# jedbrown/spectral-petsc

Measured on NVIDIA B200. Metric: spectral MatMult GDOF/s (fp64), higher is better.
Workload: dtype f64

## Files before the change

### spectral_petsc_b200/csrc/elliptic.cu

```cuda
#include "elliptic.h"

#include <algorithm>
#include <cmath>
#include <cstdlib>
#include <vector>

#include "../../include/spectral_b200.h"
#include "cheb_matrix.h"
#include "common.cuh"
#include "deriv.h"

namespace sb200 {

namespace {

struct LineInfo {
  bool interior;
  long long gid0;
  long long did0;
};

__device__ __forceinline__ LineInfo decode_line(const GridDesc& gd, long long line) {
  const int d = gd.d, PL = gd.dim[d - 1];
  long long rem = line, cnt = -gd.goff;
// ... 169 lines not shown
int GridDesc::init_slab(int d_, const int* dim_global, int rank, int nranks) {
  SB_TRY(init(d_, dim_global));
  if (nranks == 1) return 0;
  SB_CHECK(d >= 2, SB200_ERR_USER, "slab partition needs at least two axes");
  SB_CHECK(dim[0] % nranks == 0, SB200_ERR_USER, "slab partition: the outermost extent must be divisible by the number of ranks");
  const int nloc = dim[0] / nranks;
  n0g = dim[0];
  i0 = rank * nloc;
  dim[0] = nloc;
  m = (long long)nloc * stride[0];
  const int lo = i0 < 1 ? 1 : i0, hi = (i0 + nloc > n0g - 1) ? n0g - 1 : i0 + nloc;
  g = (long long)(hi > lo ? hi - lo : 0) * istride[0];
  goff = (long long)(lo - 1) * istride[0];
  return 0;
}

int EllipticCtx::create(int d, const int* dim, int rank, int nranks, EllipticCtx** out) {
  EllipticCtx* e = new EllipticCtx();
  int rc = e->init(d, dim, rank, nranks);
  if (rc) {
    delete e;
    return rc;
  }
  *out = e;
  return 0;
}

int EllipticCtx::init(int d, const int* dim, int rank, int nranks) {
  SB_TRY(gd.init_slab(d, dim, rank, nranks));
  gtot = 1;
  for (int k = 0; k < d; k++) {
    gdim[k] = dim[k];
    gtot *= dim[k] - 2;
  }
  nw = 2 + d;
  const size_t mb = (size_t)gd.m * sizeof(double);
  const int narr = nw + d + 2 + (nranks > 1 ? 6 : 0);
  SB_TRY(arena.init((size_t)narr * (mb + 256), rank, nranks));
  for (int k = 0; k < nw; k++) SB_CHECK((w[k] = arena.alloc_doubles(gd.m)), SB200_ERR_CUDA, "arena exhausted");
  for (int k = 0; k < d; k++) {
    SB_CHECK((gradu[k] = arena.alloc_doubles(gd.m)), SB200_ERR_CUDA, "arena exhausted");
    SB_CUDA(cudaMemset(gradu[k], 0, mb));
  }
  SB_CHECK((eta = arena.alloc_doubles(gd.m)), SB200_ERR_CUDA, "arena exhausted");
  SB_CHECK((deta = arena.alloc_doubles(gd.m)), SB200_ERR_CUDA, "arena exhausted");
  if (nranks > 1) {
    SB_CHECK((eta_p = arena.alloc_doubles(gd.m)), SB200_ERR_CUDA, "arena exhausted");
    SB_CHECK((deta_p = arena.alloc_doubles(gd.m)), SB200_ERR_CUDA, "arena exhausted");
    SB_CHECK((g0_p = arena.alloc_doubles(gd.m)), SB200_ERR_CUDA, "arena exhausted");
    SB_CHECK((Wp = arena.alloc_doubles(gd.m)), SB200_ERR_CUDA, "arena exhausted");
    SB_CHECK((Xp = arena.alloc_doubles(gd.m)), SB200_ERR_CUDA, "arena exhausted");
    SB_CHECK((Yp = arena.alloc_doubles(gd.m)), SB200_ERR_CUDA, "arena exhausted");
  }
  SB_CUDA(cudaMalloc((void**)&sync, 512));
  SB_CUDA(cudaMemset(sync, 0, 512));
  SB_CUDA(cudaMalloc((void**)&dirichlet, std::max<size_t>(8, (size_t)(gd.m - gd.g) * sizeof(double))));
  SB_CUDA(cudaMemset(dirichlet, 0, std::max<size_t>(8, (size_t)(gd.m - gd.g) * sizeof(double))));
  SB_CUDA(cudaMalloc((void**)&b, std::max<size_t>(8, (size_t)gd.g * sizeof(double))));
  SB_CUDA(cudaMemset(b, 0, std::max<size_t>(8, (size_t)gd.g * sizeof(double))));
  {
    std::vector<double> ones((size_t)gd.m, 1.0);
    SB_CUDA(cudaMemcpy(eta, ones.data(), mb, cudaMemcpyHostToDevice));
    SB_CUDA(cudaMemset(deta, 0, mb));
  }
  for (int k = 0; k < d; k++) {
    Dax[k] = nullptr;
    for (int q = 0; q < k; q++)
      if (gdim[q] == gdim[k]) Dax[k] = Dax[q];
    if (!Dax[k]) {
      DiffMatrix* dm = new DiffMatrix();
      SB_TRY(DiffMatrix::create(gdim[k], dm));
      owned.push_back(dm);
      Dax[k] = dm;
    }
  }
  return 0;
}

EllipticCtx::~EllipticCtx() {
  free_slab_maps(tmaps);
  arena.destroy();
  if (dirichlet) cudaFree(dirichlet);
  if (b) cudaFree(b);
  if (sync) cudaFree(sync);
  if (gexec) {
    cudaDeviceSynchronize();
    cudaGraphExecDestroy(gexec);
  }
  if (gstream) cudaStreamDestroy(gstream);
  if (gU) cudaFree(gU);
  if (gV) cudaFree(gV);
  for (DiffMatrix* dm : owned) {
    dm->destroy();
    delete dm;
  }
}

bool EllipticCtx::fusable() const {
  static int use = -1;
  if (use < 0) {
    const char* c = getenv("SB200_NO_EO");
    const char* f = getenv("SB200_NO_FUSE");
    use = ((c && atoi(c)) || (f && atoi(f))) ? 0 : 1;
  }
  if (!use || arena.nranks > 1 || gd.d > SB200_EO_MAX_JOBS) return false;
  for (int k = 0; k < gd.d; k++)
    if (!deriv_eo_supported(job(k, w[0], w[1], nullptr, DERIV_STORE))) return false;
  return true;
// ... 66 lines not shown
  p.O = gd.m / (gd.stride[axis] * gd.dim[axis]);
  p.R = gd.stride[axis];
  p.xs = p.ys = 1;
  p.xoff = p.yoff = 0;
  p.mode = mode;
  if (axis == 0 && arena.nranks > 1) {
    SB_CHECK(arena.attached(), SB200_ERR_USER, "slab partition: peers are not attached (exchange the IPC handles first)");
    if (slab_deriv0_pencil_supported(arena, p)) return slab_deriv0_pencil(arena, p, gd.dim[0], gd.i0, Xp, Yp, s);
    p.npeer = arena.nranks;
    p.nloc = gd.dim[0];
    p.row0 = gd.i0;
    for (int q = 0; q < arena.nranks; q++) p.xpeer[q] = arena.on(q, x);
    SB_TRY(arena.barrier(s));
    SB_TRY(deriv_apply(p, s));
    return arena.barrier(s);
  }
  return deriv_apply(p, s);
}

int EllipticCtx::pad(const double* U, bool with_dirichlet, double* local, cudaStream_t s) {
  const int PL = gd.dim[gd.d - 1];
  const long long nlines = gd.m / PL;
  const int tx = 32;
  dim3 blk(tx, 256 / tx);
  pad_kernel<<<(unsigned)((nlines + blk.y - 1) / blk.y), blk, 0, s>>>(gd, nlines, U, with_dirichlet ? dirichlet : nullptr, local);
  count_launch();
  SB_CUDA(cudaGetLastError());
  return 0;
}

int EllipticCtx::crop(const double* local, const double* rhs, double* V, cudaStream_t s) {
  const int PL = gd.dim[gd.d - 1];
  const long long nlines = gd.m / PL;
  const int tx = PL >= 128 ? 128 : (PL > 32 ? 64 : 32);
  dim3 blk(tx, 256 / tx);
  crop_kernel<<<(unsigned)((nlines + blk.y - 1) / blk.y), blk, 0, s>>>(gd, nlines, local, rhs, V);
  count_launch();
  SB_CUDA(cudaGetLastError());
  return 0;
}

int EllipticCtx::matmult(const double* U, double* V, cudaStream_t s) {
  SB_CHECK(U && V && U != V, SB200_ERR_ARG, "MatMult_Elliptic: U and V must be distinct non-null vectors");
  if (arena.nranks > 1) {
    SB_CHECK(arena.attached(), SB200_ERR_USER, "slab partition: peers are not attached (exchange the IPC handles first)");
    SB_CHECK(!arena.failed(), SB200_ERR_CUDA, "slab partition: a device-side flag wait timed out earlier (a peer never arrived or the ranks' calls went out of step); results are undefined, the context refuses further work");
    if ((path == 0 || path == 3) && elliptic_slab_fused_supported(*this)) {
      last_kernel = "slab step: stage_kernel + persist_kernel<P,8,1,SLAB> per rank (axis-0 chain on pencils exchanged through NVLink peer memory)";
      return elliptic_matmult_slab_fused(*this, U, V, s);
    }
    SB_CHECK(path <= 1, SB200_ERR_SUP, "slab partition: the fused path needs equal extents P in {32,64,128}");
  } else if (path == 3 || (path == 0 && elliptic_persist_supported(*this))) {
    SB_CHECK(elliptic_persist_supported(*this), SB200_ERR_SUP, "persistent path needs equal extents P % 16 == 0 between 32 and 160");
    last_kernel = "persist_kernel<P,NWARPS,1> phases A+B (the whole MatMult step: 2 PDL-linked launches)";
    return elliptic_matmult_persist(*this, U, V, s);
  }
  if (path == 2 && arena.nranks == 1) {
    SB_CHECK(elliptic_fused_supported(*this), SB200_ERR_SUP, "fused path needs equal extents P in {32,64,128}");
    last_kernel = "chain_kernel per axis";
    return elliptic_matmult_fused(*this, U, V, s);
  }
  if (path == 4 && arena.nranks == 1) {
    last_kernel = "generic path replayed from a CUDA graph";
    return matmult_graph(U, V, s);
  }
  last_kernel = "generic path: pad + per-axis deriv_kernel / eo_deriv_kernel + pointwise kernels";
  return matmult_generic(U, V, s);
}

int EllipticCtx::matmult_graph(const double* U, double* V, cudaStream_t s) {
  const size_t bytes = (size_t)gd.g * sizeof(double);
  if (!gexec) {
    if (!gU) SB_CUDA(cudaMalloc((void**)&gU, bytes));
    if (!gV) SB_CUDA(cudaMalloc((void**)&gV, bytes));
    if (!gstream) SB_CUDA(cudaStreamCreateWithFlags(&gstream, cudaStreamNonBlocking));
    SB_CUDA(cudaStreamSynchronize(s));
    SB_CUDA(cudaMemsetAsync(gU, 0, bytes, gstream));
    SB_TRY(matmult_generic(gU, gV, gstream));
    SB_CUDA(cudaStreamSynchronize(gstream));
    SB_CUDA(cudaStreamBeginCapture(gstream, cudaStreamCaptureModeThreadLocal));
    const int rc = matmult_generic(gU, gV, gstream);
    cudaGraph_t graph = nullptr;
    const cudaError_t ce = cudaStreamEndCapture(gstream, &graph);
    if (rc || ce != cudaSuccess || !graph) {
      if (graph) cudaGraphDestroy(graph);
      cudaGetLastError();
      SB_CHECK(rc == 0, rc, "MatMult_Elliptic: the generic path failed while being captured");
      set_last_error(std::string("cudaStreamEndCapture: ") + cudaGetErrorString(ce));
      return SB200_ERR_CUDA;
    }
    size_t nn = 0;
    cudaGraphGetNodes(graph, nullptr, &nn);
    gnodes = (int)nn;
    const cudaError_t ie = cudaGraphInstantiate(&gexec, graph, 0);
    cudaGraphDestroy(graph);
    SB_CUDA(ie);
  }
  SB_CUDA(cudaMemcpyAsync(gU, U, bytes, cudaMemcpyDeviceToDevice, s));
  SB_CUDA(cudaGraphLaunch(gexec, s));
  SB_CUDA(cudaMemcpyAsync(V, gV, bytes, cudaMemcpyDeviceToDevice, s));
  count_launch(gnodes);
  return 0;
}

int EllipticCtx::matmult_generic(const double* U, double* V, cudaStream_t s) {
  const int d = gd.d;
  if (fusable()) {
// ... 69 lines not shown
```

### spectral_petsc_b200/csrc/elliptic.h

```cpp
#pragma once
#include <cuda_runtime.h>

#include <vector>

#include "symm.h"

#define SB200_MAX_DIM 10
#define SB200_EO_MAX_P 160

namespace sb200 {

struct DiffMatrix {
  int P = 0, Pp = 0;
  double* d_D = nullptr;
  double* d_Ae = nullptr;
  double* d_Bo = nullptr;
  int HP = 0;
  double* d_Aep = nullptr;
  double* d_Bop = nullptr;
  static int create(int P, DiffMatrix* out);
  void destroy();
};

struct GridDesc {
  int d;
  int dim[SB200_MAX_DIM];
  long long stride[SB200_MAX_DIM];
  long long istride[SB200_MAX_DIM];
  long long m, g;
  int i0, n0g;
  long long goff;
  int init(int d, const int* dim);
  int init_slab(int d, const int* dim_global, int rank, int nranks);
  __host__ __device__ int gext(int j) const { return j == 0 ? n0g : dim[j]; }
  __host__ __device__ int gidx(int j, int i) const { return j == 0 ? i + i0 : i; }
};

struct EllipticCtx {
  GridDesc gd;
  int nw = 0;
  double* w[SB200_MAX_DIM + 2] = {};
  double* gradu[SB200_MAX_DIM] = {};
  double* eta = nullptr;
  double* deta = nullptr;
  double* dirichlet = nullptr;
  double* b = nullptr;
  double gamma = 0.0, exponent = 2.0;
  int path = 0;
  const char* last_kernel = "none";
  long long* trace = nullptr;
  unsigned* sync = nullptr;
  DiffMatrix* Dax[SB200_MAX_DIM] = {};
  std::vector<DiffMatrix*> owned;
  SymmArena arena;
  int gdim[SB200_MAX_DIM] = {};
  long long gtot = 0;
  double* Wp = nullptr;
  double* eta_p = nullptr;
  double* deta_p = nullptr;
  double* g0_p = nullptr;
  double* Xp = nullptr;
  double* Yp = nullptr;
  bool pencil_valid = false;
  unsigned long long mm_epoch = 0;
  struct SlabMaps* tmaps = nullptr;
  bool tmaps_tried = false;

  static int create(int d, const int* dim, int rank, int nranks, EllipticCtx** out);
  int init(int d, const int* dim, int rank, int nranks);
  ~EllipticCtx();
  int refresh_pencils(cudaStream_t s);
  int deriv(int axis, const double* x, double* y, const double* yin, int mode, cudaStream_t s);
  bool fusable() const;
  struct EoLineMap line_map(int axis) const;
  struct DerivParams job(int axis, const double* x, double* y, const double* yin, int mode) const;
// ... 25 lines not shown
```

### spectral_petsc_b200/csrc/elliptic_persist.cu

```cuda
#include <cstdlib>

#include "../../include/spectral_b200.h"
#include "chain.cuh"
#include "deriv.h"
#include "elliptic.h"
#include "persist.h"

#ifdef SB200_ABLATE
#define XF(p, bit) (((p).xflags & (bit)) != 0)
#else
#define XF(p, bit) false
#endif

#ifdef SB200_TRACE
#define STAMP(k) do { if (lane == 0 && p.trace) tr[k] = clock64(); } while (0)
#else
#define STAMP(k) do { } while (0)
#endif

namespace sb200 {

namespace {

__device__ __forceinline__ unsigned long long gtime() {
  unsigned long long t;
  asm volatile("mov.u64 %0, %%globaltimer;" : "=l"(t));
  return t;
}
__device__ __forceinline__ void tl_stamp(const PersistParams& p, int slot) {
  if (!XF(p, 64) || p.epoch != p.tl_epoch) return;
  unsigned long long* ts = reinterpret_cast<unsigned long long*>(p.sync) + 16;
  const unsigned long long t = gtime();
  atomicMin(ts + 2 * slot, t);
  atomicMax(ts + 2 * slot + 1, t);
}


template <int P, int NT, bool RIGHT>
__device__ __forceinline__ void load_item(double* Xw, const double* __restrict__ U, int d, int axis,
                                          long long n0, int lane, const SlabGeom sg) {
  constexpr int BE = RIGHT ? EO<P>::BLOCK_ELEMS_RIGHT : EO<P>::BLOCK_ELEMS_LEFT;
#pragma unroll
  for (int j = 0; j < NT; j++) load_block_from_U<P, RIGHT>(Xw + j * BE, U, d, axis, (unsigned)(n0 + 8 * j), lane, sg);
}

struct FluxBuf {
  double2 e[2][2], de[2][2], gg[2][2];
};

template <int P, bool RIGHT>
__device__ __forceinline__ void flux_load(FluxBuf& f, const Own<P, RIGHT>& own, int ib, const double* __restrict__ eta,
                                          const double* __restrict__ deta, const double* __restrict__ g0) {
#pragma unroll
  for (int ii = 0; ii < 2; ii++) {
    if (ib + ii >= EO<P>::MT) continue;
    if (eta == nullptr) {
      f.e[ii][0] = f.e[ii][1] = make_double2(1.5, 1.5);
      f.de[ii][0] = f.de[ii][1] = f.gg[ii][0] = f.gg[ii][1] = make_double2(0.25, 0.25);
      continue;
    }
    const long long ot = own.top(ib + ii), ob = own.bot(ib + ii);
    f.e[ii][0] = ldg2(eta + ot);
    f.e[ii][1] = ldg2(eta + ob);
    f.de[ii][0] = ldg2(deta + ot);
    f.de[ii][1] = ldg2(deta + ob);
    f.gg[ii][0] = ldg2(g0 + ot);
    f.gg[ii][1] = ldg2(g0 + ob);
  }
}

template <int P, bool RIGHT>
__device__ __forceinline__ void flux_apply(const FluxBuf& f, const Own<P, RIGHT>& own, int ib, double* Xj,
                                           const double (&a)[EO<P>::MT][2], const double (&b)[EO<P>::MT][2]) {
#pragma unroll
  for (int ii = 0; ii < 2; ii++) {
    const int i = ib + ii;
    if (i >= EO<P>::MT) continue;
    const int st = own.stop(i), sb = own.sbot(i);
    const double2 wt = ld2(Xj + st), wb = ld2(Xj + sb);
    const double yt0 = a[i][0] + b[i][0], yt1 = a[i][1] + b[i][1];
    const double yb0 = RIGHT ? b[i][1] - a[i][1] : b[i][0] - a[i][0];
    const double yb1 = RIGHT ? b[i][0] - a[i][0] : b[i][1] - a[i][1];
    const double ft0 = __dadd_rn(__dmul_rn(f.e[ii][0].x, yt0), __dmul_rn(__dmul_rn(f.de[ii][0].x, wt.x), f.gg[ii][0].x));
    const double ft1 = __dadd_rn(__dmul_rn(f.e[ii][0].y, yt1), __dmul_rn(__dmul_rn(f.de[ii][0].y, wt.y), f.gg[ii][0].y));
    const double fb0 = __dadd_rn(__dmul_rn(f.e[ii][1].x, yb0), __dmul_rn(__dmul_rn(f.de[ii][1].x, wb.x), f.gg[ii][1].x));
    const double fb1 = __dadd_rn(__dmul_rn(f.e[ii][1].y, yb1), __dmul_rn(__dmul_rn(f.de[ii][1].y, wb.y), f.gg[ii][1].y));
    st2(Xj + st, ft0, ft1);
    st2(Xj + sb, fb0, fb1);
  }
}

__device__ __forceinline__ void tma_store_2d(const CUtensorMap* map, int c0, int c1, const void* smem_src) {
  const unsigned s = (unsigned)__cvta_generic_to_shared(smem_src);
  asm volatile("cp.async.bulk.tensor.2d.global.shared::cta.bulk_group [%0, {%1, %2}], [%3];" ::"l"(map), "r"(c0), "r"(c1), "r"(s) : "memory");
}

struct NoEarly {
  __device__ __forceinline__ void operator()() const {}
};

template <int P, int NT, bool RIGHT, bool DEEP, bool PENCIL = false, bool WAITDONE = false, typename F = NoEarly>
__device__ __forceinline__ void run_item(const PersistParams& p, int axis, long long n0, const double* Ae,
                                         const double* Bo, double* Xw, int lane, const SlabMaps* maps = nullptr, double* stage = nullptr,
                                         F after_gemm2 = F()) {
  using E = EO<P>;
  static_assert(!(PENCIL && RIGHT), "pencil items are strided-axis items");
  constexpr int BE = RIGHT ? E::BLOCK_ELEMS_RIGHT : E::BLOCK_ELEMS_LEFT;
  const int g = lane >> 2, t = lane & 3;
  LineGeom lg;
  lg.R = PENCIL ? p.Rp : p.R[axis];
  lg.PR = (long long)P * lg.R;
  lg.nlines = PENCIL ? p.Rp : p.nlines;
  Own<P, RIGHT> own[NT];
  long long base0[NT];
#pragma unroll
  for (int j = 0; j < NT; j++) {
    const long long nj = n0 + 8 * j;
    base0[j] = RIGHT ? nj * P : lg.base(nj);
    own[j].base = RIGHT ? (nj + g) * P : base0[j] + 2 * t;
    own[j].R = lg.R;
    own[j].g = g;
    own[j].t = t;
  }
  const double* __restrict__ g0 = PENCIL ? p.g0_p : p.g0[axis];
  const double* __restrict__ eta_a = PENCIL ? p.eta_p : p.eta;
  const double* __restrict__ deta_a = PENCIL ? p.deta_p : p.deta;
  const double* __restrict__ etap = XF(p, 1) ? nullptr : eta_a;
#ifdef SB200_TRACE
  long long* tr = p.trace ? p.trace + ((long long)axis * (p.nlines / (8 * NT)) + n0 / (8 * NT)) * 8 : nullptr;
  if (lane == 0 && p.trace) { unsigned smid; asm("mov.u32 %0, %%smid;" : "=r"(smid)); tr[6] = smid; tr[7] = threadIdx.x >> 5; }
#endif
  STAMP(0);
  FluxBuf f0, f1;
  if (DEEP) flux_load<P, RIGHT>(f0, own[0], 0, etap, deta_a, g0);
#pragma unroll
  for (int j = 0; j < NT; j++) {
    prefetch_block<P, RIGHT>(eta_a, base0[j], lg.R, lane);
    prefetch_block<P, RIGHT>(deta_a, base0[j], lg.R, lane);
    prefetch_block<P, RIGHT>(g0, base0[j], lg.R, lane);
    if (RIGHT && !PENCIL) {
      for (int k = 0; k < p.d - 1; k++) prefetch_block<P, true>(p.part[k], base0[j], 1, lane);
    }
  }
  cp_async_wait<0>();
  __syncwarp();
  STAMP(1);

  double a[NT][E::MT][2], b[NT][E::MT][2];
  eo_gemm_nt<P, NT, RIGHT>(Ae, Bo, Xw, a, b, g, t);
// ... 20 lines not shown
    }
  }
  __syncwarp();
  STAMP(3);
  eo_gemm_nt<P, NT, RIGHT>(Ae, Bo, Xw, a, b, g, t);
  __syncwarp();
  after_gemm2();
  STAMP(4);

  if (XF(p, 2)) {
    if (a[0][0][0] + b[0][0][0] == 12345.678) p.V[0] = 1.0;
  } else if (PENCIL && NT == 1 && p.bulk) {
    asm volatile("cp.async.bulk.wait_group.read 0;" ::: "memory");
    __syncwarp();
#pragma unroll
    for (int i = 0; i < E::MT; i++) {
      const int mt = i * 8 + g, mb = P - 1 - mt;
      st2(stage + mt * 8 + 2 * t, a[0][i][0] + b[0][i][0], a[0][i][1] + b[0][i][1]);
      st2(stage + mb * 8 + 2 * t, b[0][i][0] - a[0][i][0], b[0][i][1] - a[0][i][1]);
    }
    asm volatile("fence.proxy.async.shared::cta;" ::: "memory");
    __syncwarp();
    if (lane < p.nranks) {
      const int nloc = 1 << p.lognloc;
      const int col = (int)((long long)p.rank * p.Rp + n0);
      tma_store_2d(&maps->m[lane], col, 0, stage + (lane << p.lognloc) * 8);
    }
    asm volatile("cp.async.bulk.commit_group;" ::: "memory");
  } else if (PENCIL) {
    const int nloc = 1 << p.lognloc;
#pragma unroll
    for (int j = 0; j < NT; j++) {
      const long long col = (long long)p.rank * p.Rp + n0 + 8 * j + 2 * t;
#pragma unroll
      for (int i = 0; i < E::MT; i++) {
        const int mt = i * 8 + g, mb = P - 1 - mt;
        const int qt = XF(p, 16) ? p.rank : mt >> p.lognloc, qb = XF(p, 16) ? p.rank : mb >> p.lognloc;
        st2(p.part0peer[qt] + (long long)(mt - qt * nloc) * p.R0 + col, a[j][i][0] + b[j][i][0], a[j][i][1] + b[j][i][1]);
        st2(p.part0peer[qb] + (long long)(mb - qb * nloc) * p.R0 + col, b[j][i][0] - a[j][i][0], b[j][i][1] - a[j][i][1]);
      }
    }
  } else if (!RIGHT) {
    double* __restrict__ part = p.part[axis];
#pragma unroll
    for (int j = 0; j < NT; j++) {
#pragma unroll
      for (int i = 0; i < E::MT; i++) {
        st2(part + own[j].top(i), a[j][i][0] + b[j][i][0], a[j][i][1] + b[j][i][1]);
        st2(part + own[j].bot(i), b[j][i][0] - a[j][i][0], b[j][i][1] - a[j][i][1]);
      }
    }
  } else {
    asm volatile("griddepcontrol.wait;" ::: "memory");
    if (WAITDONE && p.merged) {
      if (lane == 0) {
        const long long t0 = clock64();
        while (*reinterpret_cast<volatile unsigned*>(p.sync + 6) < p.nlocal_items) {
          if (clock64() - t0 > SB200_SPIN_LIMIT) {
            symm_record_timeout(p.sf.f[p.rank]);
            break;
          }
        }
        __threadfence();
      }
      __syncwarp();
    }
    if (WAITDONE && !XF(p, 8)) {
      if (lane == 0) tl_stamp(p, 6);
      if (lane < p.nranks) spin_until(p.sf.f[p.rank] + SYMM_DONE + lane, p.epoch, p.sf.f[p.rank]);
      __syncwarp();
      if (lane == 0) tl_stamp(p, 7);
    }
#pragma unroll
    for (int j = 0; j < NT; j++) {
      long long n = n0 + 8 * j + g, gid = 0, mul = 1;
      bool vint = true;
      for (int q = p.d - 2; q >= 0; q--) {
        int iq;
        if (q == 0) {
          iq = (int)n + p.sg.i0;
        } else {
          iq = (int)(n % P);
          n /= P;
        }
        const int ext = q == 0 ? p.sg.n0g : P;
        vint = vint && iq > 0 && iq < ext - 1;
        gid += (long long)(iq - 1) * mul;
        mul *= P - 2;
      }
      const long long vrow = gid * (P - 2) - p.sg.goff - 1;
#pragma unroll
      for (int ib = 0; ib < E::MT; ib += 4) {
        double2 ot[4], ob[4];
#pragma unroll
        for (int ii = 0; ii < 4; ii++) ot[ii] = ob[ii] = make_double2(0.0, 0.0);
        if (p.d == 3) {
          double2 lt[2][4], lb[2][4];
#pragma unroll
          for (int k = 0; k < 2; k++) {
            const double* __restrict__ pk = p.part[k];
#pragma unroll
            for (int ii = 0; ii < 4; ii++) {
              if (ib + ii >= E::MT) continue;
              lt[k][ii] = __ldcg(reinterpret_cast<const double2*>(pk + own[j].top(ib + ii)));
              lb[k][ii] = __ldcg(reinterpret_cast<const double2*>(pk + own[j].bot(ib + ii)));
            }
// ... 69 lines not shown
      const bool live = line < l1;
      const unsigned ml = line / lpp, lin = line - ml * lpp;
      unsigned rem = lin;
      long long gid = 0, ist = P - 2;
      bool inter = live;
      for (int j = d - 2; j >= 1; j--) {
        const int ij = (int)(rem % P);
        rem /= P;
        inter = inter && ij >= 1 && ij <= P - 2;
        gid += (long long)(ij - 1) * ist;
        ist *= (P - 2);
      }
      const int i0g = (int)ml + p.sg.i0;
      inter = inter && i0g >= 1 && i0g <= p.sg.n0g - 2;
      gid += (long long)(i0g - 1) * ist - p.sg.goff;
#pragma unroll
      for (int it = 0; it < IT; it++) {
        const int k = 2 * lane + 64 * it;
        v[b][it][0] = (inter && k >= 1 && k <= P - 2) ? U[gid + k - 1] : 0.0;
        v[b][it][1] = (inter && k + 1 <= P - 2) ? U[gid + k] : 0.0;
        const unsigned n = lin * P + k, q = n / Rp;
        dst[b][it] = (live && k < P) ? p.wppeer[q] + (long long)i0g * Rp + (n - q * Rp) : nullptr;
      }
    }
#pragma unroll
    for (int b = 0; b < LB; b++)
#pragma unroll
      for (int it = 0; it < IT; it++)
        if (dst[b][it]) st2(dst[b][it], v[b][it][0], v[b][it][1]);
  }
}

template <int P>
__global__ void __launch_bounds__(128, 6) stage_kernel(PersistParams p) {
  asm volatile("griddepcontrol.launch_dependents;" ::: "memory");
  stage_push_share<P>(p, threadIdx.x >> 5, blockDim.x >> 5);
  if (threadIdx.x == 0) tl_stamp(p, 1);
  __syncthreads();
  if (threadIdx.x == 0) {
    __threadfence_system();
    tl_stamp(p, 2);
    if (atomicAdd(p.sync + 3, 1u) == gridDim.x - 1) {
      p.sync[3] = 0;
      __threadfence_system();
      for (int q = 0; q < p.nranks; q++) st_relaxed_sys(p.sf.f[q] + SYMM_READY + p.rank, p.epoch);
    }
  }
}

constexpr int persist_maxreg(int nwarps, bool slab_a) {
  return nwarps > 8 ? (65536 / (nwarps * 32)) / 8 * 8 : (slab_a ? 216 : 255);
}

template <int P, int NWARPS, int NT, bool LASTPHASE, bool SLAB>
__global__ void __maxnreg__(persist_maxreg(NWARPS, SLAB && !LASTPHASE)) persist_kernel(PersistParams p, const __grid_constant__ SlabMaps maps) {
  using E = EO<P>;
  extern __shared__ __align__(128) double sm[];
  double* Ae = sm;
  double* Bo = sm + E::H * E::LDM;
  constexpr int BEMAX = E::BLOCK_ELEMS_RIGHT > E::BLOCK_ELEMS_LEFT ? E::BLOCK_ELEMS_RIGHT : E::BLOCK_ELEMS_LEFT;
  const int warp = threadIdx.x >> 5, lane = threadIdx.x & 31;
  double* Xw = sm + E::MAT_ELEMS + warp * (NT * BEMAX);
  double* stage = (SLAB && !LASTPHASE) ? sm + E::MAT_ELEMS + NWARPS * (NT * BEMAX) + warp * (P * 8) : nullptr;
  unsigned* sync = p.sync + (LASTPHASE ? 4 : 0);

  const unsigned items_per_axis = (unsigned)(p.nlines / (8 * NT));
  const unsigned items0 = (SLAB && !LASTPHASE) ? (unsigned)(p.Rp / (8 * NT)) : 0u;
  const unsigned nlocal = LASTPHASE ? items_per_axis : items_per_axis * (p.d - 1 - p.first_axis);
  const bool merged = SLAB && !LASTPHASE && p.merged;
  const unsigned total = nlocal + items0 + (merged ? items_per_axis : 0u);
  if (!LASTPHASE) asm volatile("griddepcontrol.launch_dependents;" ::: "memory");

  load_matrices<P>(sm, p.Ae, p.Bo);
  if (SLAB && threadIdx.x == 0) tl_stamp(p, LASTPHASE ? 5 : 0);

  const unsigned nstatic = gridDim.x * NWARPS;
  auto grab = [&]() -> unsigned {
    unsigned tk = 0;
    if (lane == 0) tk = atomicAdd(sync, 1u) + nstatic;
    return __shfl_sync(0xffffffffu, tk, 0);
  };
  const unsigned first_ticket = warp * gridDim.x + blockIdx.x;
  bool peers_ready = false;
  auto issue_load = [&](unsigned tk) {
    if (tk >= total) return;
    if (SLAB && !LASTPHASE && tk >= nlocal + items0) {
      load_item<P, NT, true>(Xw, p.U, p.d, p.d - 1, (long long)(tk - nlocal - items0) * (8 * NT), lane, p.sg);
      return;
    }
    if (SLAB && !LASTPHASE && tk >= nlocal) {
      if (!peers_ready && !XF(p, 4)) {
        if (lane < p.nranks) spin_until(p.sf.f[p.rank] + SYMM_READY + lane, p.epoch, p.sf.f[p.rank]);
        __syncwarp();
        if (lane == 0) tl_stamp(p, 3);
        peers_ready = true;
      }
      LineGeom lg;
      lg.R = p.Rp;
      lg.PR = (long long)P * p.Rp;
      lg.nlines = p.Rp;
#pragma unroll
      for (int j = 0; j < NT; j++)
        load_block<P, false>(Xw + j * E::BLOCK_ELEMS_LEFT, p.Wp, lg, (long long)(tk - nlocal) * (8 * NT) + 8 * j, lane);
      return;
    }
    const unsigned tl = tk;
    const int arel = LASTPHASE ? 0 : tl / items_per_axis;
    const int axis = LASTPHASE ? p.d - 1 : p.first_axis + arel;
    const long long n0 = (long long)(tl - arel * items_per_axis) * (8 * NT);
    load_item<P, NT, LASTPHASE>(Xw, p.U, p.d, axis, n0, lane, p.sg);
  };

  constexpr bool DEEP = (NWARPS * NT <= 8);
  unsigned tk = 0;
  if (SLAB && !LASTPHASE) {
    cp_async_wait<0>();
    __syncthreads();
    tk = first_ticket;
    issue_load(tk);
  } else {
    tk = first_ticket;
    issue_load(tk);
    cp_async_wait<0>();
    __syncthreads();
  }
  if (p.stagger > 0) {
    const long long until = clock64() + (long long)(warp / 4) * p.stagger;
    while (clock64() < until) {
    }
  }

  unsigned pencil_done = 0;
  auto report_pencils = [&]() {
    if (p.bulk) {
      asm volatile("cp.async.bulk.wait_group 0;" ::: "memory");
      asm volatile("fence.proxy.async.global;" ::: "memory");
      __syncwarp();
    }
    __threadfence_system();
    if (lane == 0) {
      const unsigned before = atomicAdd(sync + 2, pencil_done);
      if (before + pencil_done == items0) {
        tl_stamp(p, 4);
        sync[2] = 0;
        __threadfence_system();
        for (int q = 0; q < p.nranks; q++) st_relaxed_sys(p.sf.f[q] + SYMM_DONE + p.rank, p.epoch);
      }
    }
    pencil_done = 0;
  };
  unsigned nxt = 0;
  while (tk < total) {
    if (SLAB && !LASTPHASE && tk >= nlocal + items0) {
      if (pencil_done) report_pencils();
      run_item<P, NT, true, DEEP, false, true>(p, p.d - 1, (long long)(tk - nlocal - items0) * (8 * NT), Ae, Bo, Xw, lane);
    } else if (SLAB && !LASTPHASE && tk >= nlocal) {
      run_item<P, NT, false, DEEP, true>(p, 0, (long long)(tk - nlocal) * (8 * NT), Ae, Bo, Xw, lane, &maps, stage);
      pencil_done++;
    } else {
      const unsigned tl = tk;
      const int arel = LASTPHASE ? 0 : tl / items_per_axis;
      const int axis = LASTPHASE ? p.d - 1 : p.first_axis + arel;
      const long long n0 = (long long)(tl - arel * items_per_axis) * (8 * NT);
      if (SLAB) {
        run_item<P, NT, LASTPHASE, DEEP, false, SLAB && LASTPHASE>(p, axis, n0, Ae, Bo, Xw, lane);
      } else {
        auto early = [&]() {
          nxt = grab();
          issue_load(nxt);
        };
        run_item<P, NT, LASTPHASE, DEEP, false, false>(p, axis, n0, Ae, Bo, Xw, lane, nullptr, nullptr, early);
      }
      if (merged) {
        __threadfence();
        __syncwarp();
        if (lane == 0) atomicAdd(sync + 6, 1u);
      }
    }
    if (SLAB) {
      tk = grab();
      issue_load(tk);
    } else {
      tk = nxt;
    }
  }
  cp_async_wait<0>();
  if (SLAB && !LASTPHASE && pencil_done) report_pencils();
  if (lane == 0) {
    const unsigned gone = atomicAdd(sync + 1, 1u);
    if (gone == gridDim.x * NWARPS - 1) {
      sync[0] = 0;
      sync[1] = 0;
      if (merged) sync[6] = 0;
      if (SLAB) tl_stamp(p, LASTPHASE ? 9 : 8);
    }
  }
}

template <int P, int NWARPS, int NT, bool LASTPHASE, bool SLAB>
int launch_phase(const PersistParams& p, size_t smem, int sms, cudaStream_t s) {
  auto kern = persist_kernel<P, NWARPS, NT, LASTPHASE, SLAB>;
  static bool attr[64] = {};
  int cur = 0;
  cudaGetDevice(&cur);
  if (!attr[cur & 63]) {
    SB_CUDA(cudaFuncSetAttribute(kern, cudaFuncAttributeMaxDynamicSharedMemorySize, (int)smem));
    attr[cur & 63] = true;
  }
  long long items = p.nlines / (8 * NT) * (LASTPHASE ? 1 : p.d - 1 - p.first_axis);
  if (SLAB && !LASTPHASE) items += p.Rp / (8 * NT) + (p.merged ? p.nlines / (8 * NT) : 0);
  if (items <= 0) return 0;
  long long grid = items < sms ? items : sms;
  if (const char* mc = getenv("SB200_MAX_CTAS")) {
    const int lim = atoi(mc);
    if (lim > 0 && grid > lim) grid = lim;
  }
  if (grid < 1) grid = 1;
  cudaLaunchConfig_t cfg = {};
  cfg.gridDim = dim3((unsigned)grid);
  cfg.blockDim = dim3(NWARPS * 32);
  cfg.dynamicSmemBytes = smem;
  cfg.stream = s;
  cudaLaunchAttribute at[1];
  at[0].id = cudaLaunchAttributeProgrammaticStreamSerialization;
  at[0].val.programmaticStreamSerializationAllowed = 1;
  cfg.attrs = at;
  cfg.numAttrs = (LASTPHASE || SLAB) ? 1 : 0;
  static const SlabMaps no_maps = {};
  SB_CUDA(cudaLaunchKernelEx(&cfg, kern, p, (SLAB && p.maps) ? *p.maps : no_maps));
  count_launch();
  return 0;
}

template <int P, int NWARPS, int NT>
int run_cfg(PersistParams& p, cudaStream_t s) {
  using E = EO<P>;
  constexpr int BEMAX = E::BLOCK_ELEMS_RIGHT > E::BLOCK_ELEMS_LEFT ? E::BLOCK_ELEMS_RIGHT : E::BLOCK_ELEMS_LEFT;
  const size_t smem = (size_t)(E::MAT_ELEMS + NWARPS * NT * BEMAX) * sizeof(double);
  const size_t smem_slab_a = smem + (size_t)NWARPS * P * 8 * sizeof(double);
  int dev = 0, sms = 148;
  cudaGetDevice(&dev);
  cudaDeviceGetAttribute(&sms, cudaDevAttrMultiProcessorCount, dev);
  if (p.nranks > 1) {
    if (!XF(p, 32)) {
      int blocks = sms;
      if (const char* mc = getenv("SB200_MAX_CTAS")) blocks = atoi(mc) > 0 ? atoi(mc) : blocks;
      {
        static bool carve[64] = {};
        if (!carve[dev & 63]) {
          cudaFuncSetAttribute(stage_kernel<P>, cudaFuncAttributePreferredSharedMemoryCarveout, cudaSharedmemCarveoutMaxShared);
          carve[dev & 63] = true;
        }
      }
      stage_kernel<P><<<blocks, 128, 0, s>>>(p);
      count_launch();
      SB_CUDA(cudaGetLastError());
    }
    p.nlocal_items = (unsigned)(p.nlines / (8 * NT) * (p.d - 1 - p.first_axis));
    if (NT != 1) p.bulk = 0;
    SB_TRY((launch_phase<P, NWARPS, NT, false, true>(p, smem_slab_a, sms, s)));
    if (!p.merged) SB_TRY((launch_phase<P, NWARPS, NT, true, true>(p, smem, sms, s)));
    return 0;
  }
  SB_TRY((launch_phase<P, NWARPS, NT, false, false>(p, smem, sms, s)));
  SB_TRY((launch_phase<P, NWARPS, NT, true, false>(p, smem, sms, s)));
  return 0;
}

}

bool elliptic_persist_supported(const EllipticCtx& e) {
  const int d = e.gd.d;
  if (d < 2 || e.arena.nranks > 1) return false;
  const int P = e.gd.dim[0];
  for (int j = 1; j < d; j++)
    if (e.gd.dim[j] != P) return false;
  return P % 16 == 0 && P >= 32 && P <= 160 && (e.gd.m / P) % 16 == 0;
}

int persist_run(int P, PersistParams& p, cudaStream_t s) {
  static int cfg = -1, stg = -1;
  if (cfg < 0) {
    const char* c = getenv("SB200_PERSIST_CFG");
    cfg = c ? atoi(c) : -1;
    const char* g = getenv("SB200_STAGGER");
    stg = g ? atoi(g) : 6000;
  }
  p.stagger = stg;
#ifdef SB200_ABLATE
  const char* xf = getenv("SB200_XFLAGS");
  p.xflags = xf ? atoi(xf) : 0;
#else
  p.xflags = 0;
#endif
  SB_CHECK(p.nlines % 16 == 0, SB200_ERR_SUP, "persistent path: line count must be a multiple of 16");
  switch (P) {
    case 32: return run_cfg<32, 16, 1>(p, s);
    case 64: return run_cfg<64, 16, 1>(p, s);
    case 48: SB_CHECK(p.nranks == 1, SB200_ERR_SUP, "persistent path: this extent is a single-GPU instantiation"); return run_cfg<48, 16, 1>(p, s);
    case 80: SB_CHECK(p.nranks == 1, SB200_ERR_SUP, "persistent path: this extent is a single-GPU instantiation"); return run_cfg<80, 12, 1>(p, s);
    case 96: SB_CHECK(p.nranks == 1, SB200_ERR_SUP, "persistent path: this extent is a single-GPU instantiation"); return run_cfg<96, 12, 1>(p, s);
    case 112: SB_CHECK(p.nranks == 1, SB200_ERR_SUP, "persistent path: this extent is a single-GPU instantiation"); return run_cfg<112, 12, 1>(p, s);
    case 144: SB_CHECK(p.nranks == 1, SB200_ERR_SUP, "persistent path: this extent is a single-GPU instantiation"); return run_cfg<144, 8, 1>(p, s);
    case 160: SB_CHECK(p.nranks == 1, SB200_ERR_SUP, "persistent path: this extent is a single-GPU instantiation"); return run_cfg<160, 8, 1>(p, s);
    case 128:
      switch (cfg >= 0 ? cfg : (p.nranks > 1 ? 2 : 1)) {
        case 0: return run_cfg<128, 16, 1>(p, s);
        case 1:
          if (p.nranks > 1) return run_cfg<128, 8, 1>(p, s);
          return run_cfg<128, 12, 1>(p, s);
        case 3: return run_cfg<128, 8, 2>(p, s);
        default: return run_cfg<128, 8, 1>(p, s);
      }
  }
  set_last_error("persistent path: unsupported extent");
  return SB200_ERR_SUP;
}

int elliptic_matmult_persist(EllipticCtx& e, const double* U, double* V, cudaStream_t s) {
  const int P = e.gd.dim[0], d = e.gd.d;
  if (!e.sync) {
    SB_CUDA(cudaMalloc((void**)&e.sync, 512));
    SB_CUDA(cudaMemsetAsync(e.sync, 0, 512, s));
  }
  PersistParams p = {};
  p.Ae = e.Dax[0]->d_Ae;
  p.Bo = e.Dax[0]->d_Bo;
  p.U = U;
  p.eta = e.eta;
  p.deta = e.deta;
  p.V = V;
  p.nlines = e.gd.m / P;
  p.d = d;
  for (int k = 0; k < d; k++) {
    p.g0[k] = e.gradu[k];
    p.part[k] = e.w[1 + k];
    p.R[k] = e.gd.stride[k];
  }
  p.sync = e.sync;
  p.sg.i0 = 0;
  p.sg.n0g = P;
  p.sg.goff = 0;
  p.first_axis = 0;
  p.nranks = 1;
  p.rank = 0;
  p.trace = e.trace;
  return persist_run(P, p, s);
}

}
```

### spectral_petsc_b200/csrc/elliptic_slab.cu

```cuda
#include <cstdlib>

#include "../../include/spectral_b200.h"
#include "common.cuh"
#include "deriv.h"
#include "elliptic.h"
#include "persist.h"

namespace sb200 {

namespace {

struct PeerPtrs {
  const double* x[SB200_MAX_RANKS];
};

__global__ void slab_to_pencil_kernel(PeerPtrs pp, double* __restrict__ xp, int P, int nloc, long long R0, long long Rp,
                                      int rank) {
  const long long total = (long long)P * Rp, stride = (long long)gridDim.x * blockDim.x;
  for (long long i = (long long)blockIdx.x * blockDim.x + threadIdx.x; i < total; i += stride) {
    const int m = (int)(i / Rp);
    const long long nl = i - (long long)m * Rp;
    const int q = m / nloc;
    xp[i] = __ldcg(pp.x[q] + (long long)(m - q * nloc) * R0 + (long long)rank * Rp + nl);
  }
// ... 26 lines not shown
  }
  return true;
}

int ilog2(int v) {
  int l = 0;
  while ((1 << l) < v) l++;
  return l;
}

}

int slab_to_pencil(const SymmArena& a, const double* x_slab, double* x_pencil, int P, long long R0, cudaStream_t s) {
  PeerPtrs pp;
  for (int q = 0; q < SB200_MAX_RANKS; q++) pp.x[q] = q < a.nranks ? a.on(q, x_slab) : nullptr;
  const long long Rp = R0 / a.nranks, total = (long long)P * Rp;
  long long blocks = (total + 255) / 256;
  if (blocks > 148 * 8) blocks = 148 * 8;
  slab_to_pencil_kernel<<<(unsigned)blocks, 256, 0, s>>>(pp, x_pencil, P, P / a.nranks, R0, Rp, a.rank);
  count_launch();
  SB_CUDA(cudaGetLastError());
  return 0;
}

int EllipticCtx::refresh_pencils(cudaStream_t s) {
  SB_TRY(arena.barrier(s));
  const int P = gdim[0];
  SB_TRY(slab_to_pencil(arena, eta, eta_p, P, gd.stride[0], s));
  SB_TRY(slab_to_pencil(arena, deta, deta_p, P, gd.stride[0], s));
  SB_TRY(slab_to_pencil(arena, gradu[0], g0_p, P, gd.stride[0], s));
  pencil_valid = true;
  return 0;
}

void free_slab_maps(SlabMaps* m) { delete m; }

bool elliptic_slab_fused_supported(const EllipticCtx& e) {
  const int d = e.gd.d, G = e.arena.nranks;
  if (G < 2 || d < 2) return false;
  const int P = e.gdim[0];
  for (int j = 1; j < d; j++)
    if (e.gdim[j] != P) return false;
  if (!(P == 32 || P == 64 || P == 128)) return false;
  if ((G & (G - 1)) != 0 || P % G != 0) return false;
  const long long R0 = e.gd.stride[0];
  if (R0 % G != 0 || (R0 / G) % 16 != 0) return false;
  return (e.gd.m / P) % 16 == 0;
}

int elliptic_matmult_slab_fused(EllipticCtx& e, const double* U, double* V, cudaStream_t s) {
  SB_CHECK(e.arena.attached(), SB200_ERR_USER, "slab partition: peers are not attached (exchange the IPC handles first)");
  const int P = e.gdim[0], d = e.gd.d, G = e.arena.nranks;
  if (!e.sync) {
    SB_CUDA(cudaMalloc((void**)&e.sync, 512));
    SB_CUDA(cudaMemsetAsync(e.sync, 0, 512, s));
  }
  if (!e.pencil_valid) SB_TRY(e.refresh_pencils(s));
  const unsigned long long epoch = ++e.mm_epoch;
  SymmFlags sf;
  for (int q = 0; q < SB200_MAX_RANKS; q++) sf.f[q] = q < G ? e.arena.flags(q) : nullptr;
  sf.rank = e.arena.rank;
  sf.nranks = G;
  PersistParams p = {};
  p.Ae = e.Dax[0]->d_Ae;
  p.Bo = e.Dax[0]->d_Bo;
  p.U = U;
  p.eta = e.eta;
  p.deta = e.deta;
  p.V = V;
  p.nlines = e.gd.m / P;
  p.d = d;
  for (int k = 0; k < d; k++) {
    p.g0[k] = e.gradu[k];
    p.part[k] = e.w[1 + k];
    p.R[k] = e.gd.stride[k];
  }
  p.sync = e.sync;
  p.sg.i0 = e.gd.i0;
  p.sg.n0g = e.gd.n0g;
  p.sg.goff = e.gd.goff;
  p.first_axis = 1;
  p.nranks = G;
  p.rank = e.arena.rank;
  const int nloc = P / G;
  p.lognloc = ilog2(nloc);
  for (int q = 0; q < G; q++) {
    p.part0peer[q] = e.arena.on(q, e.w[1]);
    p.wppeer[q] = e.arena.on(q, e.Wp);
  }
  p.Wp = e.Wp;
  p.eta_p = e.eta_p;
  p.deta_p = e.deta_p;
  p.g0_p = e.g0_p;
  p.R0 = e.gd.stride[0];
  p.Rp = p.R0 / G;
  p.sf = sf;
  p.epoch = epoch;
  {
    static int bulk = -1;
    if (bulk < 0) {
      const char* c = getenv("SB200_SLAB_BULK");
      bulk = c ? atoi(c) : 1;
    }
    if (bulk && !e.tmaps_tried) {
      e.tmaps_tried = true;
      e.tmaps = new SlabMaps();
      if (!encode_part0_maps(p.part0peer, G, p.R0, nloc, e.tmaps)) {
        delete e.tmaps;
// ... 28 lines not shown
```

### spectral_petsc_b200/csrc/persist.h

```cpp
#pragma once
#include <cuda.h>
#include <cuda_runtime.h>

#include "elliptic.h"

namespace sb200 {

struct SlabGeom {
  int i0, n0g;
  long long goff;
};

struct PersistParams {
  const double* Ae;
  const double* Bo;
  const double* U;
  const double* eta;
  const double* deta;
  const double* g0[SB200_MAX_DIM];
  double* part[SB200_MAX_DIM];
  double* V;
  long long R[SB200_MAX_DIM];
  long long nlines;
  int d;
  unsigned* sync;
  SlabGeom sg;
  int first_axis;
  int nranks, rank, lognloc;
  const double* Wp;
  double* wppeer[SB200_MAX_RANKS];
  double* part0peer[SB200_MAX_RANKS];
  const double* eta_p;
  const double* deta_p;
  const double* g0_p;
  long long R0, Rp;
  SymmFlags sf;
  unsigned long long epoch;
  int bulk;
  const SlabMaps* maps;
  int merged;
  unsigned nlocal_items;
  unsigned long long tl_epoch;
  int stagger;
  int xflags;
  long long* trace;
};

struct alignas(64) SlabMaps {
  CUtensorMap m[SB200_MAX_RANKS];
};

int persist_run(int P, PersistParams& p, cudaStream_t s);

}
```

Baseline: 20.79.

## Merge persistent MatMult phases into one cooperative launch with per-plane counters

For a single GPU, the persistent path now runs the whole MatMult step in one cooperative kernel launch instead of two PDL-linked phases. Last-axis work items spin-wait on device counters: one counter for the axis-0 items and one per plane for the middle axes. This lets the last-axis work begin as soon as its own plane is ready rather than after a grid-wide phase boundary. The costs are spin-wait latency, atomic counter traffic and a larger sync buffer, with a fallback to the two-launch form if the cooperative launch is too large or the extent is 160.

```diff
diff --git a/spectral_petsc_b200/csrc/elliptic.cu b/spectral_petsc_b200/csrc/elliptic.cu
--- a/spectral_petsc_b200/csrc/elliptic.cu
+++ b/spectral_petsc_b200/csrc/elliptic.cu
@@ -245,8 +245,8 @@
     SB_CHECK((Xp = arena.alloc_doubles(gd.m)), SB200_ERR_CUDA, "arena exhausted");
     SB_CHECK((Yp = arena.alloc_doubles(gd.m)), SB200_ERR_CUDA, "arena exhausted");
   }
-  SB_CUDA(cudaMalloc((void**)&sync, 512));
-  SB_CUDA(cudaMemset(sync, 0, 512));
+  SB_CUDA(cudaMalloc((void**)&sync, ELLIPTIC_SYNC_BYTES));
+  SB_CUDA(cudaMemset(sync, 0, ELLIPTIC_SYNC_BYTES));
   SB_CUDA(cudaMalloc((void**)&dirichlet, std::max<size_t>(8, (size_t)(gd.m - gd.g) * sizeof(double))));
   SB_CUDA(cudaMemset(dirichlet, 0, std::max<size_t>(8, (size_t)(gd.m - gd.g) * sizeof(double))));
   SB_CUDA(cudaMalloc((void**)&b, std::max<size_t>(8, (size_t)gd.g * sizeof(double))));
@@ -419,7 +419,8 @@
     SB_CHECK(path <= 1, SB200_ERR_SUP, "slab partition: the fused path needs equal extents P in {32,64,128}");
   } else if (path == 3 || (path == 0 && elliptic_persist_supported(*this))) {
     SB_CHECK(elliptic_persist_supported(*this), SB200_ERR_SUP, "persistent path needs equal extents P % 16 == 0 between 32 and 160");
-    last_kernel = "persist_kernel<P,NWARPS,1> phases A+B (the whole MatMult step: 2 PDL-linked launches)";
+    SB_CHECK(!arena.failed(), SB200_ERR_CUDA, "MatMult_Elliptic: a dependency wait of the persistent kernel timed out earlier; results are undefined, the context refuses further work");
+    last_kernel = "persist_kernel<P,NWARPS,1> (the whole MatMult step: 1 cooperative launch, last-axis items wait on per-plane counters)";
     return elliptic_matmult_persist(*this, U, V, s);
   }
   if (path == 2 && arena.nranks == 1) {
diff --git a/spectral_petsc_b200/csrc/elliptic.h b/spectral_petsc_b200/csrc/elliptic.h
--- a/spectral_petsc_b200/csrc/elliptic.h
+++ b/spectral_petsc_b200/csrc/elliptic.h
@@ -21,6 +21,8 @@
   static int create(int P, DiffMatrix* out);
   void destroy();
 };
+
+constexpr size_t ELLIPTIC_SYNC_BYTES = 2048;
 
 struct GridDesc {
   int d;
diff --git a/spectral_petsc_b200/csrc/elliptic_persist.cu b/spectral_petsc_b200/csrc/elliptic_persist.cu
--- a/spectral_petsc_b200/csrc/elliptic_persist.cu
+++ b/spectral_petsc_b200/csrc/elliptic_persist.cu
@@ -13,7 +13,7 @@
 #endif
 
 #ifdef SB200_TRACE
-#define STAMP(k) do { if (lane == 0 && p.trace) tr[k] = clock64(); } while (0)
+#define STAMP(k) do { if (lane == 0 && p.trace) tr[k] = gtime(); } while (0)
 #else
 #define STAMP(k) do { } while (0)
 #endif
@@ -95,6 +95,31 @@
   asm volatile("cp.async.bulk.tensor.2d.global.shared::cta.bulk_group [%0, {%1, %2}], [%3];" ::"l"(map), "r"(c0), "r"(c1), "r"(s) : "memory");
 }
 
+template <int P, int NT>
+__device__ __forceinline__ void wait_partials(const PersistParams& p, long long n0, int lane) {
+  if (lane == 0) {
+    const long long lpp = p.nlines / P;
+    const unsigned items0 = (unsigned)(p.nlines / (8 * NT));
+    const unsigned per_plane = p.d > 2 ? (unsigned)((p.d - 2) * lpp / (8 * NT)) : 0u;
+    const volatile unsigned* done0 = p.sync + SYNC_DONE0;
+    const volatile unsigned* plane = p.sync + SYNC_PLANE + (p.d > 2 ? n0 / lpp : 0);
+    if (*done0 < items0 || *plane < per_plane) {
+      const long long t0 = clock64();
+      unsigned ns = 32;
+      while (*done0 < items0 || *plane < per_plane) {
+        if (clock64() - t0 > SB200_SPIN_LIMIT) {
+          symm_record_timeout(p.sf.f[p.rank]);
+          break;
+        }
+        __nanosleep(ns);
+        if (ns < 512) ns *= 2;
+      }
+    }
+    __threadfence();
+  }
+  __syncwarp();
+}
+
 struct NoEarly {
   __device__ __forceinline__ void operator()() const {}
 };
@@ -221,6 +246,7 @@
     }
   } else {
     asm volatile("griddepcontrol.wait;" ::: "memory");
+    if (!WAITDONE && p.single) wait_partials<P, NT>(p, n0, lane);
     if (WAITDONE && p.merged) {
       if (lane == 0) {
         const long long t0 = clock64();
@@ -396,8 +422,9 @@
   return nwarps > 8 ? (65536 / (nwarps * 32)) / 8 * 8 : (slab_a ? 216 : 255);
 }
 
-template <int P, int NWARPS, int NT, bool LASTPHASE, bool SLAB>
+template <int P, int NWARPS, int NT, bool LASTPHASE, bool SLAB, bool SINGLE = false>
 __global__ void __maxnreg__(persist_maxreg(NWARPS, SLAB && !LASTPHASE)) persist_kernel(PersistParams p, const __grid_constant__ SlabMaps maps) {
+  static_assert(!SINGLE || (!SLAB && !LASTPHASE), "the one-launch form is single-GPU and has no phase B");
   using E = EO<P>;
   extern __shared__ __align__(128) double sm[];
   double* Ae = sm;
@@ -412,8 +439,9 @@
   const unsigned items0 = (SLAB && !LASTPHASE) ? (unsigned)(p.Rp / (8 * NT)) : 0u;
   const unsigned nlocal = LASTPHASE ? items_per_axis : items_per_axis * (p.d - 1 - p.first_axis);
   const bool merged = SLAB && !LASTPHASE && p.merged;
-  const unsigned total = nlocal + items0 + (merged ? items_per_axis : 0u);
-  if (!LASTPHASE) asm volatile("griddepcontrol.launch_dependents;" ::: "memory");
+  constexpr bool single = SINGLE;
+  const unsigned total = nlocal + items0 + ((merged || single) ? items_per_axis : 0u);
+  if (!LASTPHASE && !single) asm volatile("griddepcontrol.launch_dependents;" ::: "memory");
 
   load_matrices<P>(sm, p.Ae, p.Bo);
   if (SLAB && threadIdx.x == 0) tl_stamp(p, LASTPHASE ? 5 : 0);
@@ -452,7 +480,10 @@
     const int arel = LASTPHASE ? 0 : tl / items_per_axis;
     const int axis = LASTPHASE ? p.d - 1 : p.first_axis + arel;
     const long long n0 = (long long)(tl - arel * items_per_axis) * (8 * NT);
-    load_item<P, NT, LASTPHASE>(Xw, p.U, p.d, axis, n0, lane, p.sg);
+    if (SINGLE && axis == p.d - 1)
+      load_item<P, NT, true>(Xw, p.U, p.d, axis, n0, lane, p.sg);
+    else
+      load_item<P, NT, LASTPHASE>(Xw, p.U, p.d, axis, n0, lane, p.sg);
   };
 
   constexpr bool DEEP = (NWARPS * NT <= 8);
@@ -513,12 +544,18 @@
           nxt = grab();
           issue_load(nxt);
         };
-        run_item<P, NT, LASTPHASE, DEEP, false, false>(p, axis, n0, Ae, Bo, Xw, lane, nullptr, nullptr, early);
-      }
-      if (merged) {
+        if (SINGLE && axis == p.d - 1)
+          run_item<P, NT, true, DEEP>(p, axis, n0, Ae, Bo, Xw, lane, nullptr, nullptr, early);
+        else
+          run_item<P, NT, LASTPHASE, DEEP>(p, axis, n0, Ae, Bo, Xw, lane, nullptr, nullptr, early);
+      }
+      if (merged || (single && axis < p.d - 1)) {
         __threadfence();
         __syncwarp();
-        if (lane == 0) atomicAdd(sync + 6, 1u);
+        if (lane == 0) {
+          unsigned* c = merged ? sync + 6 : p.sync + (axis == 0 ? SYNC_DONE0 : SYNC_PLANE + (int)(n0 / (p.nlines / P)));
+          atomicAdd(c, 1u);
+        }
       }
     }
     if (SLAB) {
@@ -530,20 +567,23 @@
   }
   cp_async_wait<0>();
   if (SLAB && !LASTPHASE && pencil_done) report_pencils();
-  if (lane == 0) {
-    const unsigned gone = atomicAdd(sync + 1, 1u);
-    if (gone == gridDim.x * NWARPS - 1) {
+  unsigned gone = 0;
+  if (lane == 0) gone = atomicAdd(sync + 1, 1u);
+  if (__shfl_sync(0xffffffffu, gone, 0) == gridDim.x * NWARPS - 1) {
+    if (lane == 0) {
       sync[0] = 0;
       sync[1] = 0;
       if (merged) sync[6] = 0;
       if (SLAB) tl_stamp(p, LASTPHASE ? 9 : 8);
     }
-  }
-}
-
-template <int P, int NWARPS, int NT, bool LASTPHASE, bool SLAB>
+    if (single)
+      for (int i = lane; i <= (p.d > 2 ? P : 0); i += 32) p.sync[SYNC_DONE0 + i] = 0;
+  }
+}
+
+template <int P, int NWARPS, int NT, bool LASTPHASE, bool SLAB, bool SINGLE = false>
 int launch_phase(const PersistParams& p, size_t smem, int sms, cudaStream_t s) {
-  auto kern = persist_kernel<P, NWARPS, NT, LASTPHASE, SLAB>;
+  auto kern = persist_kernel<P, NWARPS, NT, LASTPHASE, SLAB, SINGLE>;
   static bool attr[64] = {};
   int cur = 0;
   cudaGetDevice(&cur);
@@ -551,7 +591,8 @@
     SB_CUDA(cudaFuncSetAttribute(kern, cudaFuncAttributeMaxDynamicSharedMemorySize, (int)smem));
     attr[cur & 63] = true;
   }
-  long long items = p.nlines / (8 * NT) * (LASTPHASE ? 1 : p.d - 1 - p.first_axis);
+  constexpr bool single = SINGLE;
+  long long items = p.nlines / (8 * NT) * (LASTPHASE ? 1 : single ? p.d : p.d - 1 - p.first_axis);
   if (SLAB && !LASTPHASE) items += p.Rp / (8 * NT) + (p.merged ? p.nlines / (8 * NT) : 0);
   if (items <= 0) return 0;
   long long grid = items < sms ? items : sms;
@@ -566,12 +607,22 @@
   cfg.dynamicSmemBytes = smem;
   cfg.stream = s;
   cudaLaunchAttribute at[1];
-  at[0].id = cudaLaunchAttributeProgrammaticStreamSerialization;
-  at[0].val.programmaticStreamSerializationAllowed = 1;
+  if (single) {
+    at[0].id = cudaLaunchAttributeCooperative;
+    at[0].val.cooperative = 1;
+  } else {
+    at[0].id = cudaLaunchAttributeProgrammaticStreamSerialization;
+    at[0].val.programmaticStreamSerializationAllowed = 1;
+  }
   cfg.attrs = at;
-  cfg.numAttrs = (LASTPHASE || SLAB) ? 1 : 0;
+  cfg.numAttrs = (single || LASTPHASE || SLAB) ? 1 : 0;
   static const SlabMaps no_maps = {};
-  SB_CUDA(cudaLaunchKernelEx(&cfg, kern, p, (SLAB && p.maps) ? *p.maps : no_maps));
+  const cudaError_t err = cudaLaunchKernelEx(&cfg, kern, p, (SLAB && p.maps) ? *p.maps : no_maps);
+  if (single && err == cudaErrorCooperativeLaunchTooLarge) {
+    cudaGetLastError();
+    return SB200_ERR_SUP;
+  }
+  SB_CUDA(err);
   count_launch();
   return 0;
 }
@@ -606,9 +657,13 @@
     if (!p.merged) SB_TRY((launch_phase<P, NWARPS, NT, true, true>(p, smem, sms, s)));
     return 0;
   }
+  if (p.single && (p.d == 2 || (p.nlines / P) % (8 * NT) == 0)) {
+    const int rc = launch_phase<P, NWARPS, NT, false, false, true>(p, smem, sms, s);
+    if (rc != SB200_ERR_SUP) return rc;
+  }
+  p.single = 0;
   SB_TRY((launch_phase<P, NWARPS, NT, false, false>(p, smem, sms, s)));
-  SB_TRY((launch_phase<P, NWARPS, NT, true, false>(p, smem, sms, s)));
-  return 0;
+  return launch_phase<P, NWARPS, NT, true, false>(p, smem, sms, s);
 }
 
 }
@@ -631,6 +686,7 @@
     stg = g ? atoi(g) : 6000;
   }
   p.stagger = stg;
+  p.single = p.nranks == 1;
 #ifdef SB200_ABLATE
   const char* xf = getenv("SB200_XFLAGS");
   p.xflags = xf ? atoi(xf) : 0;
@@ -646,7 +702,10 @@
     case 96: SB_CHECK(p.nranks == 1, SB200_ERR_SUP, "persistent path: this extent is a single-GPU instantiation"); return run_cfg<96, 12, 1>(p, s);
     case 112: SB_CHECK(p.nranks == 1, SB200_ERR_SUP, "persistent path: this extent is a single-GPU instantiation"); return run_cfg<112, 12, 1>(p, s);
     case 144: SB_CHECK(p.nranks == 1, SB200_ERR_SUP, "persistent path: this extent is a single-GPU instantiation"); return run_cfg<144, 8, 1>(p, s);
-    case 160: SB_CHECK(p.nranks == 1, SB200_ERR_SUP, "persistent path: this extent is a single-GPU instantiation"); return run_cfg<160, 8, 1>(p, s);
+    case 160:
+      SB_CHECK(p.nranks == 1, SB200_ERR_SUP, "persistent path: this extent is a single-GPU instantiation");
+      p.single = 0;
+      return run_cfg<160, 8, 1>(p, s);
     case 128:
       switch (cfg >= 0 ? cfg : (p.nranks > 1 ? 2 : 1)) {
         case 0: return run_cfg<128, 16, 1>(p, s);
@@ -664,8 +723,8 @@
 int elliptic_matmult_persist(EllipticCtx& e, const double* U, double* V, cudaStream_t s) {
   const int P = e.gd.dim[0], d = e.gd.d;
   if (!e.sync) {
-    SB_CUDA(cudaMalloc((void**)&e.sync, 512));
-    SB_CUDA(cudaMemsetAsync(e.sync, 0, 512, s));
+    SB_CUDA(cudaMalloc((void**)&e.sync, ELLIPTIC_SYNC_BYTES));
+    SB_CUDA(cudaMemsetAsync(e.sync, 0, ELLIPTIC_SYNC_BYTES, s));
   }
   PersistParams p = {};
   p.Ae = e.Dax[0]->d_Ae;
@@ -688,6 +747,9 @@
   p.first_axis = 0;
   p.nranks = 1;
   p.rank = 0;
+  p.sf.f[0] = e.arena.flags(0);
+  p.sf.rank = 0;
+  p.sf.nranks = 1;
   p.trace = e.trace;
   return persist_run(P, p, s);
 }
diff --git a/spectral_petsc_b200/csrc/elliptic_slab.cu b/spectral_petsc_b200/csrc/elliptic_slab.cu
--- a/spectral_petsc_b200/csrc/elliptic_slab.cu
+++ b/spectral_petsc_b200/csrc/elliptic_slab.cu
@@ -102,8 +102,8 @@
   SB_CHECK(e.arena.attached(), SB200_ERR_USER, "slab partition: peers are not attached (exchange the IPC handles first)");
   const int P = e.gdim[0], d = e.gd.d, G = e.arena.nranks;
   if (!e.sync) {
-    SB_CUDA(cudaMalloc((void**)&e.sync, 512));
-    SB_CUDA(cudaMemsetAsync(e.sync, 0, 512, s));
+    SB_CUDA(cudaMalloc((void**)&e.sync, ELLIPTIC_SYNC_BYTES));
+    SB_CUDA(cudaMemsetAsync(e.sync, 0, ELLIPTIC_SYNC_BYTES, s));
   }
   if (!e.pencil_valid) SB_TRY(e.refresh_pencils(s));
   const unsigned long long epoch = ++e.mm_epoch;
diff --git a/spectral_petsc_b200/csrc/persist.h b/spectral_petsc_b200/csrc/persist.h
--- a/spectral_petsc_b200/csrc/persist.h
+++ b/spectral_petsc_b200/csrc/persist.h
@@ -41,6 +41,7 @@
   int merged;
   unsigned nlocal_items;
   unsigned long long tl_epoch;
+  int single;
   int stagger;
   int xflags;
   long long* trace;
@@ -50,6 +51,10 @@
   CUtensorMap m[SB200_MAX_RANKS];
 };
 
+constexpr int SYNC_DONE0 = 128;
+constexpr int SYNC_PLANE = 129;
+static_assert((SYNC_PLANE + 160) * sizeof(unsigned) <= ELLIPTIC_SYNC_BYTES, "plane counters of the largest extent");
+
 int persist_run(int P, PersistParams& p, cudaStream_t s);
 
 }
```

Measured after the change: 22.15, median of 6. 6.6% higher.
